# achraf-15/neural_image_compression

Hardware: NVIDIA B200
Metric: 768x512 images/s (fwd+likelihood+rd terms) (higher is better)
Workload: dtype bf16x3 (bf16 hi+lo operands, f32 accumulate)

## Files before the change

neural_image_compression_b200/csrc/conv_tc.cu:

```cuda
#include <cuda.h>
#include <stdlib.h>

#include "conv_common.cuh"
#include "tc_host.cuh"
#include "tc_primitives.cuh"

namespace nic {

using namespace tc;

void set_trace_buffer(void* p);
int conv_fwd_fp32(const nic_conv_desc*, const void*, const void*, const float*, const void*, const float*, void*, void*, size_t, cudaStream_t);
int gdn_fwd_fp32(const float* x, int n, int c, int h, int w, int layout, int inverse, const float* gamma, const float* beta, float* y, cudaStream_t st);
int gdn_fwd_fp32_split(const float* x, int n, int c, int h, int w, int inverse, const float* gamma, const float* beta, void* y, cudaStream_t st);
int conv_fwd_fp32_ex(const nic_conv_desc* d, const void* x, const void* w_packed, const float* bias, void* y, int out_bf16_nhwc,
                     cudaStream_t st);

int pack_gdn_x3(int32_t c, float beta_min, const float* beta_raw, const float* gamma_raw, float* beta_eff, void* gamma_packed, cudaStream_t st);
int gdn_fwd_tc_x3(const void* x, int pair_in, long npix, int c, int inverse, const void* gamma_packed, const float* beta_eff, void* y, cudaStream_t st);
size_t packed_first_x3_elems(int cout);
int pack_first_x3(const float* w_ref, void* w_packed, int cout, cudaStream_t st);
int conv_first_x3(const nic_conv_desc* d, const void* x, const void* w_packed, const float* bias, float* y, cudaStream_t st);
int conv_first_gdn_x3(const nic_conv_desc* d, const void* x, const void* w_packed, const float* bias, const void* gamma_packed,
                      const float* beta_eff, void* y, cudaStream_t st);
// ... 84 lines not shown
                                     box_h, stride, (int)r);
  return NIC_OK;
}

int encode_2d_c32(CUtensorMap* m, const void* base, uint64_t inner, uint64_t rows, uint32_t box_rows) {
  EncodeTiledFn enc = get_encode();
  if (!enc) return fail(NIC_E_CUDA, "cuTensorMapEncodeTiled entry point not available");
  cuuint64_t dims[2] = {inner, rows};
  cuuint64_t strides[1] = {inner * 2};
  cuuint32_t box[2] = {32, box_rows};
  cuuint32_t es[2] = {1, 1};
  CUresult r = enc(m, CU_TENSOR_MAP_DATA_TYPE_BFLOAT16, 2, const_cast<void*>(base), dims, strides, box, es, CU_TENSOR_MAP_INTERLEAVE_NONE,
                   CU_TENSOR_MAP_SWIZZLE_64B, CU_TENSOR_MAP_L2_PROMOTION_L2_256B, CU_TENSOR_MAP_FLOAT_OOB_FILL_NONE);
  if (r != CUDA_SUCCESS) return fail(NIC_E_CUDA, "cuTensorMapEncodeTiled(2d %llu x %llu, 32-column box x %u) failed: %d", (unsigned long long)inner,
                                     (unsigned long long)rows, box_rows, (int)r);
  return NIC_OK;
}

int encode_nhwc_c32(CUtensorMap* m, const void* base, int n, int h, int w, int c, int box_w, int box_h) {
  EncodeTiledFn enc = get_encode();
  if (!enc) return fail(NIC_E_CUDA, "cuTensorMapEncodeTiled entry point not available");
  cuuint64_t dims[4] = {(cuuint64_t)c, (cuuint64_t)w, (cuuint64_t)h, (cuuint64_t)n};
  cuuint64_t strides[3] = {(cuuint64_t)c * 2, (cuuint64_t)w * c * 2, (cuuint64_t)h * w * c * 2};
  cuuint32_t box[4] = {32, (cuuint32_t)box_w, (cuuint32_t)box_h, 1};
  cuuint32_t es[4] = {1, 1, 1, 1};
  CUresult r = enc(m, CU_TENSOR_MAP_DATA_TYPE_BFLOAT16, 4, const_cast<void*>(base), dims, strides, box, es, CU_TENSOR_MAP_INTERLEAVE_NONE,
                   CU_TENSOR_MAP_SWIZZLE_64B, CU_TENSOR_MAP_L2_PROMOTION_L2_256B, CU_TENSOR_MAP_FLOAT_OOB_FILL_NONE);
  if (r != CUDA_SUCCESS) return fail(NIC_E_CUDA, "cuTensorMapEncodeTiled(nhwc %dx%dx%dx%d, 32-channel box %dx%d) failed: %d", n, h, w, c, box_w, box_h, (int)r);
  return NIC_OK;
}


namespace {

constexpr int kTileH = 16, kTileW = 8;
constexpr int kMaxSlots = 4;
constexpr int kMaxBSlots = 8;
constexpr int kEpiWarps = 8;
constexpr int kMmaWarps = 2;
constexpr int kFirstEpiWarp = 2 + kMmaWarps;
constexpr int kThreads = (kFirstEpiWarp + kEpiWarps) * 32;
constexpr int kMaxDynSmem = 232448 - 8192;
constexpr int kMaxCout = 1792;

struct TcTap { int8_t plane, roff, coff, slab; };
struct TcPhase {
  int8_t py, px, nplanes, pad0;
  int8_t plane_ph[4], plane_pw[4], plane_dymin[4], plane_dxmin[4];
  int8_t plane_tap_begin[5];
};

struct TcParams {
  TcPhase phases[kMaxPhases];
  TcTap taps[kMaxTaps];
  int nphases, in_stride, out_stride;
  int n, hin, win, cin, cout, hout, wout;
  int hp, wp;
  int mt;
  int blk_roff[2], blk_coff[2];
  int tile_h, tile_w;
  int tiles_x, tiles_y, n_ntiles, total_tiles;
  int b_slot_bytes;
  int pair;
  int chunk_perm;
  int tail_first, tail_n;
  int nt_inner;
  int pos_per_wave, spatial_tiles;
  int nchunks;
  int a_chunk_mod;
  const int* lo_flag;
  int split_out;
  int split_lo_off;
  int ph_rows, pw_cols;
  int slot_bytes, nsa, nsb;
  int swap;
  int b_resident;
  int nslabs;
  int nb, cout_pad;
  int epilogue;
  int out_dtype;
  long ys_n, ys_c, ys_h, ys_w;
  int flat_hw;
  int stage2;
  int tma_out;
  int out_c_offset;
  int shuffle_cout;
  int bias_mod;
  int dbg;
  long long* dbg_times;
  const float* bias;
  const float* beta;
  void* y;
  int* status;
  int off_a, off_b, off_gamma, off_sq, smem_bytes;
};

struct __align__(8) TcBarriers {
  uint64_t a_full[kMaxSlots], a_empty[kMaxSlots], b_full[kMaxBSlots], b_empty[kMaxBSlots];
  uint64_t acc_full[2], acc_empty[2], gdn_full, gamma_full, bres_full;
  uint32_t tmem_base;
  volatile int abort_flag;
};

__device__ __forceinline__ bool wait_or_abort(uint64_t* bar, uint32_t parity, TcBarriers* sb, int* status) {
  for (uint32_t i = 0; i < (1u << 22); ++i) {
    if (mbar_try_wait(bar, parity)) return true;
    if ((i & 255u) == 255u && sb->abort_flag) return false;
  }
  sb->abort_flag = 1;
  atomicExch(status, 1);
  return false;
}

__device__ __forceinline__ void trace(const TcParams& p, uint32_t tile_iter, int slot) {
  if (p.dbg_times && tile_iter < 16) {
    p.dbg_times[(static_cast<long>(blockIdx.x) * 32 + tile_iter) * 16 + slot] = clock64();
    if (slot == 0) {
      unsigned long long ns;
      asm volatile("mov.u64 %0, %%globaltimer;" : "=l"(ns));
      p.dbg_times[(static_cast<long>(blockIdx.x) * 32 + tile_iter) * 16 + 15] = static_cast<long long>(ns);
    }
  }
}

__device__ __forceinline__ bool decode_tile(const TcParams& p, int tile, int& ntile, int& phase, int& img, int& ty, int& tx) {
  if (p.pair && (p.pos_per_wave || p.n_ntiles > 1)) {
    const int V = p.nphases * p.n_ntiles;
    const int u = tile >> 1, pp = u / V, v = u - pp * V;
    int s = 2 * pp + (tile & 1);
    if (s >= p.spatial_tiles) return false;
    ntile = v % p.n_ntiles;
    phase = (v / p.n_ntiles + (p.pos_per_wave ? pp : 0)) % p.nphases;
    tx = s % p.tiles_x; s /= p.tiles_x;
    ty = s % p.tiles_y; img = s / p.tiles_y;
    return true;
  }
  if (p.pos_per_wave) {
    const int V = p.nphases * p.n_ntiles;
    int s = tile / V;
    const int v = tile - s * V;
    ntile = v % p.n_ntiles;
    phase = (v / p.n_ntiles + s) % p.nphases;
    tx = s % p.tiles_x; s /= p.tiles_x;
    ty = s % p.tiles_y; img = s / p.tiles_y;
    return true;
  }
  if (p.tail_n && tile >= p.tail_first) {
    const int k = tile - p.tail_first;
    tile = p.tail_first + (p.pair ? ((k >> 2) << 1) + (k & 1) : k >> 1);
  }
  if (p.nt_inner) {
    ntile = tile % p.n_ntiles; tile /= p.n_ntiles;
    tx = tile % p.tiles_x; tile /= p.tiles_x;
    ty = tile % p.tiles_y; tile /= p.tiles_y;
    img = tile % p.n; phase = tile / p.n;
    return true;
  }
  tx = tile % p.tiles_x; tile /= p.tiles_x;
  ty = tile % p.tiles_y; tile /= p.tiles_y;
  img = tile % p.n; tile /= p.n;
  phase = tile % p.nphases; tile /= p.nphases;
  ntile = tile;
  return true;
}

__device__ __forceinline__ int tail_block(const TcParams& p, int tile) {
// ... 204 lines not shown
        tmem_ld_32x32(gdn_addr + cg * 32, v);
        if (!KEEPX) {
          tmem_ld_32x32(acc_addr + cg * 32, xr);
          tmem_ld_wait();
#pragma unroll
          for (int j = 0; j < 32; ++j) xr[j] += s_bias[cg * 32 + j];
        } else {
          tmem_ld_wait();
        }
        const float* xp = xr + (KEEPX ? i * 32 : 0);
        if (igdn) {
#pragma unroll
          for (int j = 0; j < 32; ++j) v[j] = xp[j] * sqrt_approx(v[j] + s_beta[cg * 32 + j]);
        } else {
#pragma unroll
          for (int j = 0; j < 32; ++j) v[j] = xp[j] * rsqrt_approx(v[j] + s_beta[cg * 32 + j]);
        }
        emit_group(cg, v);
      }
    }
  } else {
    const int per = (NW == 8) ? (ncg + 1) / 2 : ncg;
    const int first = (NW == 8) ? hs * per : 0;
    const int last = (first + per < ncg) ? first + per : ncg;
    const int npass = p.split_out ? 2 : 1;
    for (int pass = 0; pass < npass; ++pass) {
      if (pass == 1) {
        fence_proxy_async_smem();
        epi_sync();
        if (leader) {
          const int wc = ox0 * p.out_stride + px, hc = oy0 * p.out_stride + py;
          for (int h = 0; h < 2; ++h)
            if (h * 64 < nvalid_c) tma_store_4d(map_o_ptr, sq + h * (128 * 128), p.out_c_offset + cbase + h * 64, wc, hc, img);
          tma_store_commit();
          if (p.stage2) tma_store_wait_read_1(); else tma_store_wait_read();
        }
        if (p.stage2) stg = sq + 2 * 128 * 128;
        epi_sync();
      }
      for (int cg = first; cg < last; ++cg) {
        float v[32];
        tmem_ld_32x32(acc_addr + cg * 32, v);
        tmem_ld_wait();
#pragma unroll
        for (int j = 0; j < 32; ++j) {
          const int c = cbase + cg * 32 + j;
          float x = v[j] + (c < p.cout ? s_bias[c] : 0.f);
          if (p.epilogue == NIC_EPI_LRELU) x = x > 0.f ? x : 0.01f * x;
          v[j] = x;
        }
        if (pass == 1) {
#pragma unroll
          for (int j = 0; j < 32; j += 2) {
            const uint32_t h = pack_bf16x2(v[j], v[j + 1]);
            v[j] -= __uint_as_float(h << 16);
            v[j + 1] -= __uint_as_float(h & 0xffff0000u);
          }
        }
        emit_group(cg, v);
      }
    }
  }
  if (leader) trace(p, trace_tile, trace_base + 4);
  if (p.tma_out) {
    fence_proxy_async_smem();
    epi_sync();
    if (leader) trace(p, trace_tile, trace_base + 5);
    if (leader && !(p.dbg & 2)) {
      const int wc = ox0 * p.out_stride + px, hc = oy0 * p.out_stride + py;
      const int lo_off = p.split_out ? p.split_lo_off : 0;
      if (p.tma_out == 2) {
        for (int h = 0; h < 4; ++h)
          if (h * 32 < nvalid_c) tma_store_4d(map_o_ptr, sq + h * (128 * 128), p.out_c_offset + cbase + h * 32, wc, hc, img);
      } else {
        for (int h = 0; h < 2; ++h)
          if (h * 64 < nvalid_c) tma_store_4d(map_o_ptr, stg + h * (128 * 128), p.out_c_offset + lo_off + cbase + h * 64, wc, hc, img);
      }
      tma_store_commit();
    }
  }
  return true;
}

__device__ __forceinline__ bool epilogue_tile_swapped(const TcParams& p, const float* s_bias, uint8_t* sq, const CUtensorMap* map_o_ptr,
                                                      uint32_t acc_tmem, int q, int lane, int hs, bool leader, int img, int ty, int tx,
                                                      int py, int px, int cbase, int nblk) {
  const int c = q * 32 + lane;
  const uint32_t lane_addr = acc_tmem + (static_cast<uint32_t>(q * 32) << 16);
  const float bias = (cbase + c < p.cout) ? s_bias[cbase + c] : 0.f;
  const int nvalid_c = p.cout - cbase;
  auto epi_sync = [&]() { asm volatile("bar.sync 1, %0;" ::"n"(kEpiWarps * 32) : "memory"); };
  uint8_t* col = sq + (c >> 6) * (128 * 128) + (c & 7) * 2;
  const uint32_t cchunk = static_cast<uint32_t>((c & 63) >> 3);
  const int npass = p.split_out ? 2 : 1;
  if (p.split_out && p.stage2) {
    for (int h = 0; h < nblk; ++h) {
      const int oy0 = ty * p.tile_h + p.blk_roff[h], ox0 = tx * p.tile_w + p.blk_coff[h];
      const int wc = ox0 * p.out_stride + px, hc = oy0 * p.out_stride + py;
      uint32_t whi[32], wlo[32];
#pragma unroll
      for (int g2 = 0; g2 < 2; ++g2) {
        float v[32];
        tmem_ld_32x32(lane_addr + h * 128 + hs * 64 + g2 * 32, v);
        tmem_ld_wait();
#pragma unroll
        for (int j = 0; j < 32; j += 2) {
          float a = v[j] + bias, b = v[j + 1] + bias;
          if (p.epilogue == NIC_EPI_LRELU) { a = a > 0.f ? a : 0.01f * a; b = b > 0.f ? b : 0.01f * b; }
          const uint32_t w = pack_bf16x2(a, b);
          whi[g2 * 16 + (j >> 1)] = w;
          wlo[g2 * 16 + (j >> 1)] = pack_bf16x2(a - __uint_as_float(w << 16), b - __uint_as_float(w & 0xffff0000u));
        }
      }
      if (leader) tma_store_wait_read();
      epi_sync();
#pragma unroll
      for (int i = 0; i < 32; ++i) {
        const int ra = hs * 64 + 2 * i, rb = ra + 1;
        uint8_t* pa = col + ra * 128 + ((cchunk ^ (ra & 7)) << 4);
        uint8_t* pb = col + rb * 128 + ((cchunk ^ (rb & 7)) << 4);
        *reinterpret_cast<uint16_t*>(pa) = static_cast<uint16_t>(whi[i] & 0xffffu);
        *reinterpret_cast<uint16_t*>(pb) = static_cast<uint16_t>(whi[i] >> 16);
        *reinterpret_cast<uint16_t*>(pa + 2 * 128 * 128) = static_cast<uint16_t>(wlo[i] & 0xffffu);
        *reinterpret_cast<uint16_t*>(pb + 2 * 128 * 128) = static_cast<uint16_t>(wlo[i] >> 16);
      }
      fence_proxy_async_smem();
      epi_sync();
      if (leader && !(p.dbg & 2)) {
        const int off = p.out_c_offset + cbase;
        for (int k = 0; k < 2; ++k)
          if (k * 64 < nvalid_c) {
            tma_store_4d(map_o_ptr, sq + k * (128 * 128), off + k * 64, wc, hc, img);
            tma_store_4d(map_o_ptr, sq + (2 + k) * (128 * 128), off + p.split_lo_off + k * 64, wc, hc, img);
          }
        tma_store_commit();
      }
    }
    return true;
  }
  for (int h = 0; h < nblk; ++h) {
    const int oy0 = ty * p.tile_h + p.blk_roff[h], ox0 = tx * p.tile_w + p.blk_coff[h];
    const int wc = ox0 * p.out_stride + px, hc = oy0 * p.out_stride + py;
    for (int pass = 0; pass < npass; ++pass) {
      if (leader) tma_store_wait_read();
      epi_sync();
#pragma unroll
      for (int g2 = 0; g2 < 2; ++g2) {
        float v[32];
        tmem_ld_32x32(lane_addr + h * 128 + hs * 64 + g2 * 32, v);
        tmem_ld_wait();
        const int r0 = hs * 64 + g2 * 32;
#pragma unroll
        for (int j = 0; j < 32; j += 2) {
          float a = v[j] + bias, b = v[j + 1] + bias;
          if (p.epilogue == NIC_EPI_LRELU) { a = a > 0.f ? a : 0.01f * a; b = b > 0.f ? b : 0.01f * b; }
          uint32_t w = pack_bf16x2(a, b);
          if (pass == 1) w = pack_bf16x2(a - __uint_as_float(w << 16), b - __uint_as_float(w & 0xffff0000u));
          const int ra = r0 + j, rb = ra + 1;
          *reinterpret_cast<uint16_t*>(col + ra * 128 + ((cchunk ^ (ra & 7)) << 4)) = static_cast<uint16_t>(w & 0xffffu);
          *reinterpret_cast<uint16_t*>(col + rb * 128 + ((cchunk ^ (rb & 7)) << 4)) = static_cast<uint16_t>(w >> 16);
        }
      }
      fence_proxy_async_smem();
      epi_sync();
      if (leader && !(p.dbg & 2)) {
        const int off = p.out_c_offset + cbase + (pass == 1 ? p.split_lo_off : 0);
        for (int k = 0; k < 2; ++k)
          if (k * 64 < nvalid_c) tma_store_4d(map_o_ptr, sq + k * (128 * 128), off + k * 64, wc, hc, img);
        tma_store_commit();
      }
    }
  }
  return true;
}

template <bool PAIR>
__global__ void __launch_bounds__(kThreads, 1)
conv_tc_kernel(const __grid_constant__ CUtensorMap map_a, const __grid_constant__ CUtensorMap map_w,
               const __grid_constant__ CUtensorMap map_g, const __grid_constant__ CUtensorMap map_o, const __grid_constant__ TcParams p) {
  extern __shared__ uint8_t smem_raw[];
  uint8_t* smem = smem_raw + ((1024u - (smem_u32(smem_raw) & 1023u)) & 1023u);
  __shared__ TcBarriers sb;
  __shared__ float s_bias[kMaxCout];
  __shared__ float s_beta[128];
  __shared__ int s_tap_brow[kMaxTaps];
  __shared__ uint32_t s_tap_aoff[kMaxTaps];
  pdl_launch_dependents();
  if (threadIdx.x < kMaxTaps) {
    s_tap_brow[threadIdx.x] = p.taps[threadIdx.x].slab;
    s_tap_aoff[threadIdx.x] = static_cast<uint32_t>((p.taps[threadIdx.x].roff * p.pw_cols + p.taps[threadIdx.x].coff) * 128) >> 4;
  }
  const int warp = threadIdx.x >> 5, lane = threadIdx.x & 31;
  const bool gdn = p.epilogue == NIC_EPI_GDN || p.epilogue == NIC_EPI_IGDN;
  const uint32_t rank = PAIR ? cluster_ctarank() : 0u;
  if (threadIdx.x == 0) {
    for (int i = 0; i < kMaxSlots; ++i) { mbar_init(&sb.a_full[i], 1); mbar_init(&sb.a_empty[i], kMmaWarps); }
    for (int i = 0; i < kMaxBSlots; ++i) { mbar_init(&sb.b_full[i], 1); mbar_init(&sb.b_empty[i], kMmaWarps); }
    for (int i = 0; i < 2; ++i) { mbar_init(&sb.acc_full[i], kMmaWarps); mbar_init(&sb.acc_empty[i], PAIR ? 2 * kEpiWarps : kEpiWarps); }
    mbar_init(&sb.gdn_full, 1); mbar_init(&sb.gamma_full, 1); mbar_init(&sb.bres_full, 1);
    sb.abort_flag = 0;
    fence_barrier_init();
  }
  if (warp == 2) {
    if (PAIR) { tmem_alloc_pair(&sb.tmem_base, 512); tmem_relinquish_pair(); }
    else { tmem_alloc(&sb.tmem_base, 512); tmem_relinquish(); }
  }
  if (warp == 0 && lane == 0) { tma_prefetch_desc(&map_a); tma_prefetch_desc(&map_w); if (gdn) tma_prefetch_desc(&map_g); if (p.tma_out) tma_prefetch_desc(&map_o); }
  pdl_wait();
  for (int i = threadIdx.x; i < p.cout; i += kThreads) s_bias[i] = p.bias[p.bias_mod ? i % p.bias_mod : i];
  if (p.beta) for (int i = threadIdx.x; i < 128; i += kThreads) s_beta[i] = p.beta[i];
  int nchunks_eff = p.nchunks, skip_from = 1 << 30, skip_add = 0;
  if (p.lo_flag && __ldg(p.lo_flag) == 0) { skip_add = p.a_chunk_mod / 2; skip_from = skip_add; nchunks_eff = p.nchunks - skip_add; }
  const int nc = p.a_chunk_mod / 2, per = (skip_add ? 2 : 3);
  const bool perm = p.chunk_perm != 0;
  auto kchunk = [&](int chunk) {
    if (perm) { const int c = chunk / per, r = chunk - c * per; return r == 0 ? c : (r == 1 ? 2 * nc + c : nc + c); }
    return chunk + (chunk >= skip_from ? skip_add : 0);
  };

  tcgen05_fence_before();
  __syncthreads();
  if (PAIR) cluster_sync();
  tcgen05_fence_after();
  const uint32_t tmem = sb.tmem_base;

  const int first_tile = blockIdx.x, tile_step = gridDim.x;

  if (warp == 0) {
    if (lane == 0) {
      uint32_t it = 0;
      bool ok = true;
      const uint32_t bytes = p.ph_rows * p.pw_cols * 128;
      for (int tile = first_tile; tile < p.total_tiles && ok; tile += tile_step) {
        int ntile, phase, img, ty, tx;
        if (!decode_tile(p, tile, ntile, phase, img, ty, tx)) break;
        const TcPhase& ph = p.phases[phase];
        for (int chunk = 0; chunk < nchunks_eff && ok; ++chunk) {
          const int kc = kchunk(chunk);
          for (int pl = 0; pl < ph.nplanes; ++pl, ++it) {
            const int s = it % p.nsa;
            if (!wait_or_abort(&sb.a_empty[s], ((it / p.nsa) & 1) ^ 1, &sb, p.status)) { ok = false; break; }
            if (chunk == 0 && pl == 0) trace(p, (tile - first_tile) / tile_step, 5);
            if (chunk == nchunks_eff - 1 && pl == ph.nplanes - 1) trace(p, (tile - first_tile) / tile_step, 6);
            const int w0 = p.in_stride * (tx * p.tile_w + ph.plane_dxmin[pl]) + ph.plane_pw[pl];
            const int h0 = p.in_stride * (ty * p.tile_h + ph.plane_dymin[pl]) + ph.plane_ph[pl];
// ... 206 lines not shown
                if (two) {
                  if (live) {
                    MMA(d_tmem, f1, f_hi, g1, g_hi, idesc_use, 1);
                    MMA(d_tmem, f1 + 2, f_hi, g1 + 2, g_hi, idesc_use, 1);
                    MMA(d_tmem, f1 + 4, f_hi, g1 + 4, g_hi, idesc_use, 1);
                    MMA(d_tmem, f1 + 6, f_hi, g1 + 6, g_hi, idesc_use, 1);
                  }
                  COMMIT(&sb.b_empty[s1]);
                  COMMIT(&sb.a_empty[sa1]);
                }
              }
              __syncwarp();
              accumulate = 1;
            }
          } else
          for (int chunk = 0; chunk < nchunks && ok; ++chunk) {
            for (int pl = 0; pl < nplanes && ok; ++pl) {
              if (!mbar_try_wait(&sb.a_full[sa], pa) && !wait_or_abort(&sb.a_full[sa], pa, &sb, p.status)) { ok = false; break; }
              if (chunk == 0 && pl == 0 && lane == 0 && mw == 0) trace(p, tcount, 1);
              tcgen05_fence_after();
              const uint32_t a_slot_lo = umma_desc_lo(a_base + sa * p.slot_bytes);
              const int t_end = ph.plane_tap_begin[pl + 1];
              for (int t = ph.plane_tap_begin[pl]; t < t_end; t += 2) {
                const bool two = t + 1 < t_end;
                if (!mbar_try_wait(&sb.b_full[sbi], pb) && !wait_or_abort(&sb.b_full[sbi], pb, &sb, p.status)) { ok = false; break; }
                const uint32_t s0 = sbi;
                if (++sbi == static_cast<uint32_t>(nsb)) { sbi = 0; pb ^= 1; }
                uint32_t s1 = s0;
                if (two) {
                  if (!mbar_try_wait(&sb.b_full[sbi], pb) && !wait_or_abort(&sb.b_full[sbi], pb, &sb, p.status)) { ok = false; break; }
                  s1 = sbi;
                  if (++sbi == static_cast<uint32_t>(nsb)) { sbi = 0; pb ^= 1; }
                }
                tcgen05_fence_after();
                const uint32_t b_lo0 = b_base_lo + s0 * bslot16, b_lo1 = b_base_lo + s1 * bslot16;
                const uint32_t a_lo0 = a_slot_lo + s_tap_aoff[t] + blk_off, a_lo1 = a_slot_lo + s_tap_aoff[two ? t + 1 : t] + blk_off;
                const uint32_t f0 = swp ? b_lo0 : a_lo0, g0 = swp ? a_lo0 : b_lo0, f1 = swp ? b_lo1 : a_lo1, g1 = swp ? a_lo1 : b_lo1;
                if (elect_one()) {
                  if (live) {
                    MMA(d_tmem, f0, f_hi, g0, g_hi, idesc_use, accumulate);
                    MMA(d_tmem, f0 + 2, f_hi, g0 + 2, g_hi, idesc_use, 1);
                    MMA(d_tmem, f0 + 4, f_hi, g0 + 4, g_hi, idesc_use, 1);
                    MMA(d_tmem, f0 + 6, f_hi, g0 + 6, g_hi, idesc_use, 1);
                  }
                  COMMIT(&sb.b_empty[s0]);
                  if (two) {
                    if (live) {
                      MMA(d_tmem, f1, f_hi, g1, g_hi, idesc_use, 1);
                      MMA(d_tmem, f1 + 2, f_hi, g1 + 2, g_hi, idesc_use, 1);
                      MMA(d_tmem, f1 + 4, f_hi, g1 + 4, g_hi, idesc_use, 1);
                      MMA(d_tmem, f1 + 6, f_hi, g1 + 6, g_hi, idesc_use, 1);
                    }
                    COMMIT(&sb.b_empty[s1]);
                  }
                }
                __syncwarp();
                accumulate = 1;
              }
              if (elect_one()) COMMIT(&sb.a_empty[sa]);
              __syncwarp();
              if (++sa == static_cast<uint32_t>(nsa)) { sa = 0; pa ^= 1; }
            }
          }
          if (lane == 0 && mw == 0) trace(p, tcount, 2);
          if (elect_one()) COMMIT(&sb.acc_full[buf]);
          __syncwarp();
        }
      }
      __syncwarp();
    }
  } else {
    const int q = warp & 3;
    uint8_t* sq = smem + p.off_sq;
    uint32_t tcount = 0, gdn_count = 0;
    bool ok = true;
    for (int tile = first_tile; tile < p.total_tiles && ok; tile += tile_step, ++tcount) {
      int ntile, phase, img, ty, tx;
      if (!decode_tile(p, tile, ntile, phase, img, ty, tx)) break;
      const TcPhase& ph = p.phases[phase];
      const int nblk = live_blocks(p, ty, tx);
      const uint32_t buf = tcount & 1;
      if (!__all_sync(0xffffffffu, wait_or_abort(&sb.acc_full[buf], (tcount >> 1) & 1, &sb, p.status))) break;
      tcgen05_fence_after();
      if (p.swap) {
        if (!(p.dbg & 8))
          ok = epilogue_tile_swapped(p, s_bias, sq, &map_o, tmem + buf * 256, q, lane, (warp - kFirstEpiWarp) >> 2,
                                     warp == kFirstEpiWarp && lane == 0, img, ty, tx, ph.py, ph.px, ntile * p.nb, nblk);
      } else
      for (int b = 0; b < nblk && ok && !(p.dbg & 8); ++b)
        if (const int only = tail_block(p, tile); only < 0 || b == only)
        ok = epilogue_block<kEpiWarps>(p, &sb, s_bias, s_beta, sq, smem + p.off_gamma, &map_o, tmem + buf * 256 + b * 128, q, lane,
                                       (warp - kFirstEpiWarp) >> 2, warp == kFirstEpiWarp && lane == 0, img, ty * p.tile_h + p.blk_roff[b],
                                       tx * p.tile_w + p.blk_coff[b], ph.py, ph.px, ntile * p.nb, gdn_count, b == 0 ? tcount : 0xffffffffu);
      if (warp == kFirstEpiWarp && lane == 0) trace(p, tcount, 4);
      tcgen05_fence_before();
      __syncwarp();
      if (lane == 0) {
        if (PAIR && rank != 0) mbar_arrive_cluster(mapa_u32(smem_u32(&sb.acc_empty[buf]), 0));
        else mbar_arrive(&sb.acc_empty[buf]);
      }
    }
    if (p.tma_out && warp == kFirstEpiWarp && lane == 0) tma_store_wait_all();
  }

  tcgen05_fence_before();
  __syncthreads();
  if (PAIR) cluster_sync();
  if (warp == 2) { if (PAIR) tmem_dealloc_pair(tmem, 512); else tmem_dealloc(tmem, 512); }
}

constexpr int kFirstThreads = 160 + 8 * 32;
constexpr int kPatchW = 20, kPatchH = 35, kPatchCols = 19, kPatchPlane = kPatchH * kPatchW;

struct FirstParams {
  const float* x;
  int n, hin, win, tiles_x, tiles_y, total_tiles;
  int off_a, off_w, off_gamma, off_sq, off_patch;
};

struct __align__(8) FirstBarriers {
  uint64_t a_full[2], a_empty[2], w_full, gdn_full2;
  TcBarriers common;
};

__global__ void __launch_bounds__(kFirstThreads, 1)
conv_first_tc_kernel(const __grid_constant__ CUtensorMap map_w, const __grid_constant__ CUtensorMap map_g,
                     const __grid_constant__ CUtensorMap map_o, const __grid_constant__ TcParams p, const __grid_constant__ FirstParams f) {
  extern __shared__ uint8_t smem_raw[];
  uint8_t* smem = smem_raw + ((1024u - (smem_u32(smem_raw) & 1023u)) & 1023u);
  __shared__ FirstBarriers fb;
  __shared__ float s_bias[128];
  __shared__ float s_beta[128];
  TcBarriers& sb = fb.common;
  const int warp = threadIdx.x >> 5, lane = threadIdx.x & 31, tid = threadIdx.x;
  if (tid < 128) { s_bias[tid] = p.bias[tid]; s_beta[tid] = p.beta[tid]; }
  if (tid == 0) {
    for (int i = 0; i < 2; ++i) {
      mbar_init(&fb.a_full[i], 128); mbar_init(&fb.a_empty[i], 1);
      mbar_init(&sb.acc_full[i], 1); mbar_init(&sb.acc_empty[i], 4);
    }
    mbar_init(&fb.w_full, 1); mbar_init(&fb.gdn_full2, 1);
    mbar_init(&sb.gdn_full, 1); mbar_init(&sb.gamma_full, 1);
    sb.abort_flag = 0;
    fence_barrier_init();
  }
  if (warp == 4) { tmem_alloc(&sb.tmem_base, 512); tmem_relinquish(); }
  tcgen05_fence_before();
  __syncthreads();
  tcgen05_fence_after();
  const uint32_t tmem = sb.tmem_base;
  const int first_tile = blockIdx.x, tile_step = gridDim.x;
  float* patch = reinterpret_cast<float*>(smem + f.off_patch);

  auto tile_coords = [&](int tile, int& img, int& ty, int& tx) {
    tx = tile % f.tiles_x; tile /= f.tiles_x; ty = tile % f.tiles_y; img = tile / f.tiles_y;
  };

  if (warp < 4) {
    auto fetch_patch = [&](int tile, int bufi) {
      int img, ty, tx;
      tile_coords(tile, img, ty, tx);
      const int y0 = 2 * (ty * 16) - 2, x0 = 2 * (tx * 8) - 2;
      const int gx = x0 + lane;
      const bool col_ok = lane < kPatchCols && gx >= 0 && gx < f.win;
      const float* base = f.x + static_cast<long>(img) * 3 * f.hin * f.win + (col_ok ? gx : 0);
      const uint32_t dst0 = smem_u32(patch + bufi * (3 * kPatchPlane)) + lane * 4;
      if (lane < kPatchCols) {
#pragma unroll
        for (int c = 0; c < 3; ++c) {
#pragma unroll
          for (int j = 0; j < 9; ++j) {
            const int yy = warp + 4 * j;
            if (yy < kPatchH) {
              const int gy = y0 + yy;
              const bool ok = col_ok && gy >= 0 && gy < f.hin;
              const float* src = base + (static_cast<long>(c) * f.hin + (ok ? gy : 0)) * f.win;
              asm volatile("cp.async.ca.shared.global [%0], [%1], 4, %2;" ::"r"(dst0 + (c * kPatchPlane + yy * kPatchW) * 4), "l"(src),
                           "r"(ok ? 4 : 0)
                           : "memory");
            }
          }
        }
      }
// ... 303 lines not shown
    if (int rc = check_first_layer(d)) return rc;
    pack_first_bf16_kernel<<<64, 256, 0, st>>>(w_ref, static_cast<__nv_bfloat16*>(w_packed));
    return check_launch("pack_first_bf16_kernel");
  }
  if (subpixel_form(d)) {
    if (d->c_in % 64) return fail(NIC_E_UNSUPPORTED, "conv bf16: c_in=%d must be a multiple of 64", d->c_in);
    const long total = 9L * 16 * d->c_in;
    pack_weight_subpixel_bf16_kernel<<<static_cast<int>((total + 255) / 256), 256, 0, st>>>(w_ref, static_cast<__nv_bfloat16*>(w_packed), d->c_in,
                                                                                         d->c_out, tt);
    return check_launch("pack_weight_subpixel_bf16_kernel");
  }
  if (d->c_in % 64) return fail(NIC_E_UNSUPPORTED, "conv bf16: c_in=%d must be a multiple of 64 (or < 64 for the first layer)", d->c_in);
  const int nb = nb_for(d->c_out);
  const int cout_pad = (d->c_out + nb - 1) / nb * nb;
  const long total = static_cast<long>(tt.ntaps) * cout_pad * d->c_in;
  const int blocks = static_cast<int>((total + 255) / 256 < 4096 ? (total + 255) / 256 : 4096);
  pack_weight_bf16_kernel<<<blocks, 256, 0, st>>>(w_ref, static_cast<__nv_bfloat16*>(w_packed), d->c_in, d->c_out, cout_pad, d->kh, d->kw,
                                                  d->transposed, tt);
  return check_launch("pack_weight_bf16_kernel");
}

int pack_gdn_tc(int32_t c, float beta_min, const float* beta_raw, const float* gamma_raw, float* beta_eff, void* gamma_packed,
                int32_t precision, cudaStream_t st) {
  if (precision == NIC_PREC_BF16X3) return pack_gdn_x3(c, beta_min, beta_raw, gamma_raw, beta_eff, gamma_packed, st);
  if (precision != NIC_PREC_BF16) return fail(NIC_E_UNSUPPORTED, "pack_gdn: precision %d", precision);
  const float pedestal = static_cast<float>(3.814697265625e-06 * 3.814697265625e-06);
  const float beta_bound = static_cast<float>(sqrt(static_cast<double>(beta_min) + static_cast<double>(pedestal)));
  const float gamma_bound = static_cast<float>(sqrt(static_cast<double>(pedestal)));
  pack_gdn_bf16_kernel<<<(c * c + 255) / 256, 256, 0, st>>>(c, beta_bound, gamma_bound, pedestal, beta_raw, gamma_raw, beta_eff,
                                                            static_cast<__nv_bfloat16*>(gamma_packed));
  return check_launch("pack_gdn_bf16_kernel");
}

size_t conv_workspace_bytes_tc(const nic_conv_desc* d) {
  const bool gdn = d->epilogue == NIC_EPI_GDN || d->epilogue == NIC_EPI_IGDN;
  if (d->precision == NIC_PREC_BF16X3 && gdn) return static_cast<size_t>(d->n) * d->h_out * d->w_out * d->c_out * sizeof(float);
  return 0;
}

static int launch_tc(const nic_conv_desc* d, const TapTable& tt, const void* x, const void* w_packed, const float* bias, const void* gdn_gamma,
                     const float* gdn_beta, void* y, cudaStream_t st, const nic_conv_desc* shuffle = nullptr, const int* lo_flag = nullptr) {
  TcParams p{};
  if (int rc = build_tc_geometry(d, tt, &p)) return rc;
  const bool gdn = d->epilogue == NIC_EPI_GDN || d->epilogue == NIC_EPI_IGDN;
  const bool x3 = d->precision == NIC_PREC_BF16X3;
  if (d->in_layout != NIC_LAYOUT_NHWC || d->in_dtype != (x3 ? NIC_DT_BF16X2 : NIC_DT_BF16))
    return fail(NIC_E_UNSUPPORTED, "conv %s: input must be NHWC %s", x3 ? "bf16x3" : "bf16", x3 ? "bf16 pairs" : "bf16");
  if (x3 && gdn) return fail(NIC_E_UNSUPPORTED, "conv bf16x3: the conv kernel has bias / LeakyReLU epilogues only (GDN follows as gdn_x3_kernel)");
  if (d->c_in % 64) return fail(NIC_E_UNSUPPORTED, "conv bf16: c_in=%d must be a multiple of 64", d->c_in);
  if (d->c_out > kMaxCout) return fail(NIC_E_UNSUPPORTED, "conv bf16: c_out=%d exceeds the %d-entry bias table of the kernel", d->c_out, kMaxCout);
  if (gdn && (d->c_out != 128 || !gdn_gamma || !gdn_beta)) return fail(NIC_E_UNSUPPORTED, "conv bf16: the fused GDN epilogue needs c_out = 128 and packed gamma/beta");
  if ((reinterpret_cast<uintptr_t>(x) & 127) || (reinterpret_cast<uintptr_t>(w_packed) & 127)) return fail(NIC_E_BADALIGN, "conv bf16: tensors must be 128-byte aligned for TMA");
  p.n = d->n; p.hin = d->h_in; p.win = d->w_in; p.cin = d->c_in; p.cout = d->c_out; p.hout = d->h_out; p.wout = d->w_out;
  p.nb = nb_for(d->c_out);
  p.cout_pad = (d->c_out + p.nb - 1) / p.nb * p.nb;
  p.n_ntiles = p.cout_pad / p.nb;
  p.nchunks = (x3 ? 3 : 1) * d->c_in / 64;
  p.a_chunk_mod = (x3 ? 2 : 1) * d->c_in / 64;
  p.lo_flag = x3 ? lo_flag : nullptr;
  p.split_out = d->out_dtype == NIC_DT_BF16X2;
  if (p.split_out && (!x3 || d->out_layout != NIC_LAYOUT_NHWC || d->c_out % 64 || d->out_c_total % 64 || d->out_c_offset % 64))
    return fail(NIC_E_UNSUPPORTED, "conv: bf16-pair output needs the bf16x3 arm, NHWC, channel counts / offsets multiples of 64");
  p.epilogue = d->epilogue; p.out_dtype = p.split_out ? NIC_DT_BF16 : d->out_dtype;
  const int chalf = d->out_c_total ? d->out_c_total : d->c_out;
  p.split_lo_off = chalf;
  const int ctot = p.split_out ? 2 * chalf : chalf;
  if (d->out_layout == NIC_LAYOUT_NCHW) { p.ys_n = static_cast<long>(ctot) * d->h_out * d->w_out; p.ys_c = static_cast<long>(d->h_out) * d->w_out; p.ys_h = d->w_out; p.ys_w = 1; }
  else { p.ys_n = static_cast<long>(d->h_out) * d->w_out * ctot; p.ys_h = static_cast<long>(d->w_out) * ctot; p.ys_w = ctot; p.ys_c = 1; }
  const size_t esz = d->out_dtype == NIC_DT_F32 ? 4 : 2;
  p.y = static_cast<uint8_t*>(y) + static_cast<size_t>(d->out_c_offset) * p.ys_c * esz;
  if (!shuffle && p.ys_c == 1 && ((reinterpret_cast<uintptr_t>(p.y) & 15) || (ctot * esz) % 16)) return fail(NIC_E_BADALIGN, "conv bf16: NHWC output rows must be 16-byte aligned");
  p.bias = bias; p.beta = gdn_beta;
  if (shuffle) {
    if (shuffle->out_dtype != NIC_DT_F32) return fail(NIC_E_UNSUPPORTED, "conv bf16: the sub-pixel output path writes fp32");
    const int sct = shuffle->out_c_total ? shuffle->out_c_total : shuffle->c_out;
    p.shuffle_cout = shuffle->c_out; p.bias_mod = shuffle->c_out;
    if (shuffle->out_layout == NIC_LAYOUT_NCHW) { p.ys_n = static_cast<long>(sct) * shuffle->h_out * shuffle->w_out; p.ys_c = static_cast<long>(shuffle->h_out) * shuffle->w_out; p.ys_h = shuffle->w_out; p.ys_w = 1; }
    else { p.ys_n = static_cast<long>(shuffle->h_out) * shuffle->w_out * sct; p.ys_h = static_cast<long>(shuffle->w_out) * sct; p.ys_w = sct; p.ys_c = 1; }
    p.y = static_cast<uint8_t*>(y) + static_cast<size_t>(shuffle->out_c_offset) * p.ys_c * 4;
  }
  p.status = status_word();
  if (!p.status) return fail(NIC_E_CUDA, "conv bf16: cannot allocate the status word");
  { const char* e = getenv("NIC_TC_DEBUG"); p.dbg = e ? atoi(e) : 0; }
  p.dbg_times = reinterpret_cast<long long*>(g_trace_buffer);

  int gn = d->n, gh = d->h_in, gw = d->w_in;
  const bool pointwise = d->kh == 1 && d->kw == 1 && d->stride == 1 && !d->transposed;
  const long npix = static_cast<long>(d->n) * d->h_in * d->w_in;
  const bool flat = pointwise && npix % kTileW == 0;
  if (flat) {
    gn = 1; gh = static_cast<int>(npix / kTileW); gw = kTileW;
    p.flat_hw = d->h_in * d->w_in;
    p.n = 1; p.hin = gh; p.win = gw; p.hout = gh; p.wout = gw;
  }
  p.hp = (p.hout + tt.out_stride - 1) / tt.out_stride;
  p.wp = (p.wout + tt.out_stride - 1) / tt.out_stride;
  const char* swap_env = getenv("NIC_TC_SWAP");
  const bool out_bf16_tma = !shuffle && d->out_layout == NIC_LAYOUT_NHWC && p.out_dtype == NIC_DT_BF16 && p.nb == 128 && d->c_out % 64 == 0 &&
                            ctot % 8 == 0 && (reinterpret_cast<uintptr_t>(y) & 15) == 0;
  const bool swap_ok = !gdn && out_bf16_tma && (d->epilogue == NIC_EPI_BIAS || d->epilogue == NIC_EPI_LRELU);
  bool swap = swap_ok && (swap_env ? atoi(swap_env) != 0 : (tt.nphases > 1 || tt.in_stride == 1));
  bool pair = false;
  {
    const char* pair_env = getenv("NIC_TC_PAIR");
    const int tx2 = (p.wp + 2 * kTileW - 1) / (2 * kTileW), ty2 = (p.hp + kTileH - 1) / kTileH;
    const long per_phase = static_cast<long>(tx2) * ty2 * p.n;
    const bool worth = x3 && (tt.nphases == 1 || per_phase * tt.nphases >= 16 * kNumSMs);
    pair = (pair_env ? atoi(pair_env) != 0 : worth) && !gdn && !flat && p.nb == 128 && p.n_ntiles <= 2 && p.wp > kTileW && per_phase % 2 == 0 &&
           per_phase * tt.nphases >= 2 * kNumSMs && !getenv("NIC_TC_MT");
    if (pair) swap = false;
  }
  p.pair = pair ? 1 : 0;
  const bool stacked = flat || swap;
  p.mt = (stacked ? p.hp > kTileH : p.wp > kTileW) ? 2 : 1;
  {
    const long tiles2 = static_cast<long>((p.wp + (stacked ? kTileW : 2 * kTileW) - 1) / (stacked ? kTileW : 2 * kTileW)) *
                        ((p.hp + (stacked ? 2 * kTileH : kTileH) - 1) / (stacked ? 2 * kTileH : kTileH)) * p.n * tt.nphases * p.n_ntiles;
    if (tiles2 < kNumSMs / 2) p.mt = 1;
    if (const char* e = getenv("NIC_TC_MT")) { const int f = atoi(e); if (f == 1) p.mt = 1; else if (f == 2 && (stacked ? p.hp > kTileH : p.wp > kTileW)) p.mt = 2; }
  }
  if (p.mt == 1) swap = false;
  p.swap = swap ? 1 : 0;
  p.blk_roff[0] = p.blk_coff[0] = 0;
  p.blk_roff[1] = stacked ? kTileH : 0; p.blk_coff[1] = stacked ? 0 : kTileW;
  p.tile_h = stacked ? kTileH * p.mt : kTileH; p.tile_w = stacked ? kTileW : kTileW * p.mt;
  p.ph_rows += p.tile_h - kTileH; p.pw_cols += p.tile_w - kTileW;
  p.tiles_x = (p.wp + p.tile_w - 1) / p.tile_w;
  p.tiles_y = (p.hp + p.tile_h - 1) / p.tile_h;
  p.total_tiles = p.tiles_x * p.tiles_y * p.n * p.nphases * p.n_ntiles;
  p.pos_per_wave = 0; p.spatial_tiles = p.tiles_x * p.tiles_y * p.n;
  p.nt_inner = p.n_ntiles > 1 ? 1 : 0;
  if (const char* e = getenv("NIC_TC_NT_INNER")) p.nt_inner = (atoi(e) != 0 && p.n_ntiles > 1) ? 1 : 0;
  {
    static const bool interleave = !(getenv("NIC_TC_PHASE_ORDER") && atoi(getenv("NIC_TC_PHASE_ORDER")) == 0);
    const double in_bytes = static_cast<double>(d->n) * d->h_in * d->w_in * d->c_in * (x3 ? 4 : 2);
    if (interleave && in_bytes > 112e6 && p.nphases > 1 && p.total_tiles >= 16 * kNumSMs) {
      p.pos_per_wave = 1;
    }
  }
  p.tail_first = 0; p.tail_n = 0;
  {
    static const bool tail = !(getenv("NIC_TC_TAIL") && atoi(getenv("NIC_TC_TAIL")) == 0);
    const int rem = p.total_tiles % kNumSMs;
    if (tail && !p.swap && p.mt == 2 && p.n_ntiles == 1 && p.nphases == 1 && !p.pos_per_wave && !p.nt_inner && p.nb == 128 &&
        p.total_tiles > 4 * kNumSMs && rem > 0 && 2 * rem <= kNumSMs && rem % 2 == 0) {
      p.tail_first = p.total_tiles - rem; p.tail_n = rem;
      p.total_tiles = p.tail_first + 2 * rem;
    }
  }
  p.nslabs = tt.ntaps;

  p.slot_bytes = (p.ph_rows * p.pw_cols * 128 + 1023) / 1024 * 1024;
  p.out_c_offset = d->out_c_offset;
  p.tma_out = (!shuffle && d->out_layout == NIC_LAYOUT_NHWC && p.out_dtype == NIC_DT_BF16 && p.nb == 128 && d->c_out % 64 == 0 &&
               ctot % 8 == 0 && (reinterpret_cast<uintptr_t>(y) & 15) == 0) ? 1 : 0;
  if (!p.tma_out && !shuffle && !gdn && d->out_layout == NIC_LAYOUT_NHWC && p.out_dtype == NIC_DT_F32 && p.nb == 128 && d->c_out % 32 == 0 &&
      ctot % 4 == 0 && (reinterpret_cast<uintptr_t>(y) & 15) == 0 && !getenv("NIC_TC_NO_F32_TMA"))
    p.tma_out = 2;
  const int tapchunks = (tt.ntaps / tt.nphases) * p.nchunks;
  const char* st2 = getenv("NIC_TC_STAGE2");
  const bool st2_fits = 2 * p.slot_bytes + 4 * 128 * 128 + 4 * 128 * 128 + 1024 <= kMaxDynSmem;
  const bool st2_auto = p.swap && tapchunks <= 96 && tt.ntaps > tt.nphases;
  p.stage2 = (p.split_out && p.tma_out == 1 && !gdn && st2_fits &&
              (st2 ? (atoi(st2) != 0 && (p.swap || tapchunks <= 96)) : st2_auto)) ? 1 : 0;
  const int stage_bytes = p.tma_out == 2 ? 4 * 128 * 128 : ((gdn || p.tma_out) ? (p.stage2 ? 4 : 2) * 128 * 128 : 0);
  const int gdn_bytes = (gdn ? 2 * 128 * 128 : 0) + stage_bytes;
  const int bres_bytes = tt.ntaps * p.nchunks * p.nb * 128;
  p.b_resident = (p.n_ntiles == 1 && p.nb <= 16 && bres_bytes + 2 * p.slot_bytes + gdn_bytes + 1024 <= kMaxDynSmem) ? 1 : 0;
  {
    static const bool perm = !(getenv("NIC_TC_CHUNK_PERM") && atoi(getenv("NIC_TC_CHUNK_PERM")) == 0);
    p.chunk_perm = (perm && x3 && !p.b_resident) ? 1 : 0;
  }
  p.b_slot_bytes = p.pair ? 64 * 128 : 128 * 128;
  if (p.b_resident) p.lo_flag = nullptr;
  int b_bytes;
  if (p.b_resident) {
    b_bytes = (bres_bytes + 1023) / 1024 * 1024; p.nsb = 1;
    p.nsa = 4;
    while (p.nsa > 2 && p.nsa * p.slot_bytes + b_bytes + gdn_bytes + 1024 > kMaxDynSmem) --p.nsa;
  } else {
    const int bslot = p.pair ? 64 * 128 : 128 * 128;
    p.nsa = 2; p.nsb = 4;
    if (2 * p.slot_bytes + 4 * bslot + gdn_bytes + 1024 > kMaxDynSmem) {
      if (p.stage2) return fail(NIC_E_UNSUPPORTED, "conv bf16x3: internal: staging tiles do not fit");
      return fail(NIC_E_UNSUPPORTED, "conv bf16: patch of %d x %d pixels does not fit shared memory", p.ph_rows, p.pw_cols);
    }
    const bool one_tap = tt.ntaps == tt.nphases;
    if (one_tap) {
      p.nsa = 2; p.nsb = 2;
      for (;;) {
        if (p.nsa <= p.nsb && p.nsa < kMaxSlots && (p.nsa + 1) * p.slot_bytes + p.nsb * bslot + gdn_bytes + 1024 <= kMaxDynSmem) ++p.nsa;
        else if (p.nsb < kMaxBSlots && p.nsa * p.slot_bytes + (p.nsb + 1) * bslot + gdn_bytes + 1024 <= kMaxDynSmem) ++p.nsb;
        else break;
      }
    } else
    for (;;) {
      if (p.nsb < kMaxBSlots && p.nsa * p.slot_bytes + (p.nsb + 1) * bslot + gdn_bytes + 1024 <= kMaxDynSmem && p.nsb < 2 * p.nsa + 2) ++p.nsb;
      else if (p.nsa < kMaxSlots && (p.nsa + 1) * p.slot_bytes + p.nsb * bslot + gdn_bytes + 1024 <= kMaxDynSmem) ++p.nsa;
      else if (p.nsb < kMaxBSlots && p.nsa * p.slot_bytes + (p.nsb + 1) * bslot + gdn_bytes + 1024 <= kMaxDynSmem) ++p.nsb;
      else break;
    }
    {
      const char* ea = getenv("NIC_TC_NSA"); const char* eb = getenv("NIC_TC_NSB");
      const int fa = ea ? atoi(ea) : 0, fb = eb ? atoi(eb) : 0;
      if (fa || fb) {
        const int na = fa ? fa : p.nsa, nb2 = fb ? fb : p.nsb;
        if (na >= 2 && na <= kMaxSlots && nb2 >= 2 && nb2 <= kMaxBSlots && na * p.slot_bytes + nb2 * bslot + gdn_bytes + 1024 <= kMaxDynSmem) { p.nsa = na; p.nsb = nb2; }
      }
    }
    b_bytes = p.nsb * bslot;
  }
  p.off_a = 0; p.off_b = p.nsa * p.slot_bytes; p.off_gamma = p.off_b + b_bytes; p.off_sq = p.off_gamma + (gdn ? 2 * 128 * 128 : 0);
  p.smem_bytes = p.off_sq + stage_bytes + 1024;

  CUtensorMap map_a, map_w, map_g, map_o;
  if (p.split_out && !p.tma_out) return fail(NIC_E_BADALIGN, "conv bf16x3: bf16-pair output must be 16-byte aligned");
  if (int rc = encode_nhwc(&map_a, x, gn, gh, gw, (x3 ? 2 : 1) * d->c_in, p.pw_cols, p.ph_rows, tt.in_stride, 2)) return rc;
  if (int rc = encode_2d(&map_w, w_packed, static_cast<uint64_t>(x3 ? 3 : 1) * d->c_in, static_cast<uint64_t>(tt.ntaps) * p.cout_pad, 64,
                         p.pair ? p.nb / 2 : p.nb)) return rc;
  if (gdn) { if (int rc = encode_2d(&map_g, gdn_gamma, 128, 128, 64, 128)) return rc; }
  else map_g = map_w;
  if (p.tma_out) {
    const int on = flat ? 1 : d->n, oh = flat ? gh : d->h_out, ow = flat ? gw : d->w_out;
    if (int rc = encode_nhwc(&map_o, y, on, oh, ow, ctot, kTileW, kTileH, tt.out_stride, p.tma_out == 2 ? 4 : 2)) return rc;
  } else map_o = map_w;

  if (int rc = ensure_dyn_smem(reinterpret_cast<const void*>(conv_tc_kernel<false>), kMaxDynSmem)) return rc;
  if (int rc = ensure_dyn_smem(reinterpret_cast<const void*>(conv_tc_kernel<true>), kMaxDynSmem)) return rc;
  const int grid = p.total_tiles < kNumSMs ? p.total_tiles : kNumSMs;
  if (p.pair) {
    if (p.mt != 2 || p.swap || p.b_resident || grid % 2) return fail(NIC_E_UNSUPPORTED, "conv tc: CTA-pair launch with an unsupported tiling");
    if (int rc = check_cuda(launch_pdl_cluster(conv_tc_kernel<true>, grid, kThreads, p.smem_bytes, st, 2, map_a, map_w, map_g, map_o, p), "conv_tc_kernel launch")) return rc;
  } else if (int rc = check_cuda(launch_pdl(conv_tc_kernel<false>, grid, kThreads, p.smem_bytes, st, map_a, map_w, map_g, map_o, p), "conv_tc_kernel launch")) return rc;
  return check_launch("conv_tc_kernel");
}

static int launch_first(const nic_conv_desc* d, const void* x, const void* w_packed, const float* bias, const void* gdn_gamma,
                        const float* gdn_beta, void* y, cudaStream_t st) {
  if (int rc = check_first_layer(d)) return rc;
  if (d->in_layout != NIC_LAYOUT_NCHW || d->in_dtype != NIC_DT_F32) return fail(NIC_E_UNSUPPORTED, "conv bf16 (first layer): input must be the NCHW fp32 image");
  if (d->out_layout != NIC_LAYOUT_NHWC || d->out_dtype != NIC_DT_BF16 || d->out_c_total > 128) return fail(NIC_E_UNSUPPORTED, "conv bf16 (first layer): output must be NHWC bf16");
  if (!gdn_gamma || !gdn_beta) return fail(NIC_E_BADSHAPE, "conv bf16 (first layer): packed gamma / beta missing");
  if ((reinterpret_cast<uintptr_t>(y) & 127) || (reinterpret_cast<uintptr_t>(w_packed) & 127)) return fail(NIC_E_BADALIGN, "conv bf16: tensors must be 128-byte aligned for TMA");
  TcParams p{};
  p.epilogue = NIC_EPI_GDN; p.out_dtype = NIC_DT_BF16; p.nb = 128; p.cout = 128; p.tma_out = 1; p.out_stride = 1;
  p.n = d->n; p.hout = d->h_out; p.wout = d->w_out; p.hp = d->h_out; p.wp = d->w_out;
  p.bias = bias; p.beta = gdn_beta; p.y = y;
// ... 85 lines not shown
```

Measured before the change: 4489.

## Release accumulator TMEM early in epilogue and add split-output block epilogue

Adds an AccRelease helper so epilogue warps signal acc_empty as soon as the last TMEM load of a tile finishes, before staging and TMA stores, which lets the MMA warp start the next tile sooner. Adds a new split-output epilogue path that loads 64 columns per thread, writes vectorised swizzled hi/lo panels, and double-buffers the TMA stores. It also enables pair mode and stage2 staging more widely when early release is on. The cost is extra shared memory for staging and different tile pairing heuristics, which could change occupancy or scheduling.

```diff
diff --git a/neural_image_compression_b200/csrc/conv_tc.cu b/neural_image_compression_b200/csrc/conv_tc.cu
--- a/neural_image_compression_b200/csrc/conv_tc.cu
+++ b/neural_image_compression_b200/csrc/conv_tc.cu
@@ -190,6 +190,7 @@
   long ys_n, ys_c, ys_h, ys_w;
   int flat_hw;
   int stage2;
+  int epi_early;
   int tma_out;
   int out_c_offset;
   int shuffle_cout;
@@ -560,9 +561,76 @@
   return true;
 }
 
+struct AccRelease {
+  uint64_t* bar;
+  bool remote;
+  __device__ __forceinline__ void operator()(int lane) {
+    if (!bar) return;
+    tcgen05_fence_before();
+    __syncwarp();
+    if (lane == 0) {
+      if (remote) mbar_arrive_cluster(mapa_u32(smem_u32(bar), 0));
+      else mbar_arrive(bar);
+    }
+    bar = nullptr;
+  }
+};
+
+__device__ __forceinline__ void epilogue_block_split(const TcParams& p, const float* s_bias, uint8_t* sq, const CUtensorMap* map_o_ptr,
+                                                     uint32_t acc_tmem, int q, int lane, int hs, bool leader, int img, int oy0, int ox0,
+                                                     int py, int px, int cbase, AccRelease* rel) {
+  const int row = q * 32 + lane, cg0 = hs * 2;
+  const uint32_t acc_addr = acc_tmem + (static_cast<uint32_t>(q * 32) << 16);
+  auto epi_sync = [&]() { asm volatile("bar.sync 1, %0;" ::"n"(kEpiWarps * 32) : "memory"); };
+  float v[64];
+  tmem_ld_32x32(acc_addr + cg0 * 32, v);
+  tmem_ld_32x32(acc_addr + (cg0 + 1) * 32, v + 32);
+  tmem_ld_wait();
+  if (rel) (*rel)(lane);
+  uint32_t whi[32], wlo[32];
+#pragma unroll
+  for (int j = 0; j < 64; j += 2) {
+    const int c = cbase + cg0 * 32 + j;
+    float a = v[j] + (c < p.cout ? s_bias[c] : 0.f), b = v[j + 1] + (c + 1 < p.cout ? s_bias[c + 1] : 0.f);
+    if (p.epilogue == NIC_EPI_LRELU) { a = a > 0.f ? a : 0.01f * a; b = b > 0.f ? b : 0.01f * b; }
+    const uint32_t w = pack_bf16x2(a, b);
+    whi[j >> 1] = w;
+    wlo[j >> 1] = pack_bf16x2(a - __uint_as_float(w << 16), b - __uint_as_float(w & 0xffff0000u));
+  }
+  uint8_t* panel = sq + hs * (128 * 128) + row * 128;
+  auto stage = [&](uint8_t* dst, const uint32_t* w) {
+#pragma unroll
+    for (int i = 0; i < 2; ++i)
+#pragma unroll
+      for (int j = 0; j < 4; ++j) {
+        const uint32_t* s = w + i * 16 + j * 4;
+        *reinterpret_cast<uint4*>(dst + (((i * 4 + j) ^ (row & 7)) << 4)) = make_uint4(s[0], s[1], s[2], s[3]);
+      }
+  };
+  const int wc = ox0 * p.out_stride + px, hc = oy0 * p.out_stride + py;
+  const int nvalid_c = p.cout - cbase;
+  auto store = [&](int t, int off) {
+    if (p.dbg & 2) return;
+    for (int h = 0; h < 2; ++h)
+      if (h * 64 < nvalid_c) tma_store_4d(map_o_ptr, sq + (2 * t + h) * (128 * 128), p.out_c_offset + off + cbase + h * 64, wc, hc, img);
+    tma_store_commit();
+  };
+  if (leader) tma_store_wait_read_1();
+  epi_sync();
+  stage(panel, whi);
+  fence_proxy_async_smem();
+  epi_sync();
+  if (leader) { store(0, 0); tma_store_wait_read_1(); }
+  epi_sync();
+  stage(panel + 2 * 128 * 128, wlo);
+  fence_proxy_async_smem();
+  epi_sync();
+  if (leader) store(1, p.split_lo_off);
+}
+
 __device__ __forceinline__ bool epilogue_tile_swapped(const TcParams& p, const float* s_bias, uint8_t* sq, const CUtensorMap* map_o_ptr,
                                                       uint32_t acc_tmem, int q, int lane, int hs, bool leader, int img, int ty, int tx,
-                                                      int py, int px, int cbase, int nblk) {
+                                                      int py, int px, int cbase, int nblk, AccRelease* rel) {
   const int c = q * 32 + lane;
   const uint32_t lane_addr = acc_tmem + (static_cast<uint32_t>(q * 32) << 16);
   const float bias = (cbase + c < p.cout) ? s_bias[cbase + c] : 0.f;
@@ -590,6 +658,7 @@
           wlo[g2 * 16 + (j >> 1)] = pack_bf16x2(a - __uint_as_float(w << 16), b - __uint_as_float(w & 0xffff0000u));
         }
       }
+      if (rel && h == nblk - 1) (*rel)(lane);
       if (leader) tma_store_wait_read();
       epi_sync();
 #pragma unroll
@@ -639,6 +708,7 @@
           *reinterpret_cast<uint16_t*>(col + rb * 128 + ((cchunk ^ (rb & 7)) << 4)) = static_cast<uint16_t>(w >> 16);
         }
       }
+      if (rel && h == nblk - 1 && pass == npass - 1) (*rel)(lane);
       fence_proxy_async_smem();
       epi_sync();
       if (leader && !(p.dbg & 2)) {
@@ -1011,23 +1081,28 @@
       const uint32_t buf = tcount & 1;
       if (!__all_sync(0xffffffffu, wait_or_abort(&sb.acc_full[buf], (tcount >> 1) & 1, &sb, p.status))) break;
       tcgen05_fence_after();
+      AccRelease rel{&sb.acc_empty[buf], PAIR && rank != 0};
+      const int hs = (warp - kFirstEpiWarp) >> 2;
+      const bool leader = warp == kFirstEpiWarp && lane == 0;
+      const int only = tail_block(p, tile);
       if (p.swap) {
         if (!(p.dbg & 8))
-          ok = epilogue_tile_swapped(p, s_bias, sq, &map_o, tmem + buf * 256, q, lane, (warp - kFirstEpiWarp) >> 2,
-                                     warp == kFirstEpiWarp && lane == 0, img, ty, tx, ph.py, ph.px, ntile * p.nb, nblk);
+          ok = epilogue_tile_swapped(p, s_bias, sq, &map_o, tmem + buf * 256, q, lane, hs, leader, img, ty, tx, ph.py, ph.px,
+                                     ntile * p.nb, nblk, p.epi_early ? &rel : nullptr);
+      } else if (p.epi_early && p.split_out) {
+        const int lastb = only < 0 ? nblk - 1 : only;
+        for (int b = 0; b < nblk && !(p.dbg & 8); ++b)
+          if (only < 0 || b == only)
+            epilogue_block_split(p, s_bias, sq, &map_o, tmem + buf * 256 + b * 128, q, lane, hs, leader, img, ty * p.tile_h + p.blk_roff[b],
+                                 tx * p.tile_w + p.blk_coff[b], ph.py, ph.px, ntile * p.nb, b == lastb ? &rel : nullptr);
       } else
       for (int b = 0; b < nblk && ok && !(p.dbg & 8); ++b)
-        if (const int only = tail_block(p, tile); only < 0 || b == only)
+        if (only < 0 || b == only)
         ok = epilogue_block<kEpiWarps>(p, &sb, s_bias, s_beta, sq, smem + p.off_gamma, &map_o, tmem + buf * 256 + b * 128, q, lane,
-                                       (warp - kFirstEpiWarp) >> 2, warp == kFirstEpiWarp && lane == 0, img, ty * p.tile_h + p.blk_roff[b],
+                                       hs, leader, img, ty * p.tile_h + p.blk_roff[b],
                                        tx * p.tile_w + p.blk_coff[b], ph.py, ph.px, ntile * p.nb, gdn_count, b == 0 ? tcount : 0xffffffffu);
-      if (warp == kFirstEpiWarp && lane == 0) trace(p, tcount, 4);
-      tcgen05_fence_before();
-      __syncwarp();
-      if (lane == 0) {
-        if (PAIR && rank != 0) mbar_arrive_cluster(mapa_u32(smem_u32(&sb.acc_empty[buf]), 0));
-        else mbar_arrive(&sb.acc_empty[buf]);
-      }
+      if (leader) trace(p, tcount, 4);
+      rel(lane);
     }
     if (p.tma_out && warp == kFirstEpiWarp && lane == 0) tma_store_wait_all();
   }
@@ -1497,6 +1572,7 @@
   p.status = status_word();
   if (!p.status) return fail(NIC_E_CUDA, "conv bf16: cannot allocate the status word");
   { const char* e = getenv("NIC_TC_DEBUG"); p.dbg = e ? atoi(e) : 0; }
+  { const char* e = getenv("NIC_TC_EPI_EARLY"); p.epi_early = (e && atoi(e) == 0) ? 0 : 1; }
   p.dbg_times = reinterpret_cast<long long*>(g_trace_buffer);
 
   int gn = d->n, gh = d->h_in, gw = d->w_in;
@@ -1520,7 +1596,7 @@
     const char* pair_env = getenv("NIC_TC_PAIR");
     const int tx2 = (p.wp + 2 * kTileW - 1) / (2 * kTileW), ty2 = (p.hp + kTileH - 1) / kTileH;
     const long per_phase = static_cast<long>(tx2) * ty2 * p.n;
-    const bool worth = x3 && (tt.nphases == 1 || per_phase * tt.nphases >= 16 * kNumSMs);
+    const bool worth = x3 && (tt.nphases == 1 || per_phase * tt.nphases >= 16 * kNumSMs || p.epi_early);
     pair = (pair_env ? atoi(pair_env) != 0 : worth) && !gdn && !flat && p.nb == 128 && p.n_ntiles <= 2 && p.wp > kTileW && per_phase % 2 == 0 &&
            per_phase * tt.nphases >= 2 * kNumSMs && !getenv("NIC_TC_MT");
     if (pair) swap = false;
@@ -1576,8 +1652,10 @@
   const char* st2 = getenv("NIC_TC_STAGE2");
   const bool st2_fits = 2 * p.slot_bytes + 4 * 128 * 128 + 4 * 128 * 128 + 1024 <= kMaxDynSmem;
   const bool st2_auto = p.swap && tapchunks <= 96 && tt.ntaps > tt.nphases;
+  bool split_early = p.epi_early && p.split_out && p.tma_out == 1 && !gdn && !p.swap;
+  if (split_early && !st2_fits) { p.epi_early = 0; split_early = false; }
   p.stage2 = (p.split_out && p.tma_out == 1 && !gdn && st2_fits &&
-              (st2 ? (atoi(st2) != 0 && (p.swap || tapchunks <= 96)) : st2_auto)) ? 1 : 0;
+              (split_early || (st2 ? (atoi(st2) != 0 && (p.swap || tapchunks <= 96)) : st2_auto))) ? 1 : 0;
   const int stage_bytes = p.tma_out == 2 ? 4 * 128 * 128 : ((gdn || p.tma_out) ? (p.stage2 ? 4 : 2) * 128 * 128 : 0);
   const int gdn_bytes = (gdn ? 2 * 128 * 128 : 0) + stage_bytes;
   const int bres_bytes = tt.ntaps * p.nchunks * p.nb * 128;
```

After: 4616, median of 6. 1.03x the previous value.
